# babybirdprd/dia-tts-prune

Measured on AMD Instinct MI355X. Metric: audio-codec frames/sec (Dia-1.6B decode, whole job), higher is better.
Workload: dtype bf16; 1 GPU; Dia-1.6B bf16 weights, bf16 K/V, batch 1, 1890 decode steps, text bytes [98], cfg 3.0 / T 1.3 / top-p 0.95 / top-k 35, hipGraph=True; batch_per_gpu=1, parallelism=single

## Files before the change

dia-tts-prune_amd/csrc/seg.hip:

```cpp
#include "common.hpp"
#include "../../include/dia_hip.h"
#include "errors.hpp"
#include "launch.hpp"
#include "tuning.hpp"

namespace {

constexpr int SG_CUS = 256;
constexpr int SG_NCW = 7;
constexpr int SG_NT = (SG_NCW + 1) * 64;
constexpr int SG_TILES = 16;
constexpr int SG_K = 2048;
constexpr int SG_D = 2048, SG_F = 8192, SG_NQ = 3072;
constexpr int SG_S_CO = SG_D / SG_CUS / 4;
constexpr int SG_S_WI = 2 * SG_F / SG_CUS / 4;
constexpr int SG_S_WO = 8;
constexpr int SG_S_QKV = SG_NQ / SG_CUS / 4;
constexpr int SG_FIRST_WI = SG_S_CO, SG_FIRST_WO = SG_S_CO + SG_S_WI, SG_FIRST_QKV = SG_FIRST_WO + SG_S_WO;
constexpr int SG_SLOTS_FULL = SG_FIRST_QKV + SG_S_QKV;
constexpr int SG_KMAX = (SG_SLOTS_FULL + SG_NCW - 1) / SG_NCW;
constexpr int SG_MAXM = 4;

constexpr int SG_CNT_STRIDE = 16;
constexpr int SG_CNT_X1 = 0, SG_CNT_H = 8, SG_CNT_P = 16, SG_CNT_X2 = 80, SG_NCNT = 88;
constexpr size_t SG_OFF_LAUNCH = (size_t)SG_NCNT * SG_CNT_STRIDE * 4;
constexpr size_t SG_OFF_ERR = SG_OFF_LAUNCH + SG_CUS * 4;
constexpr size_t SG_CTRL_BYTES = (SG_OFF_ERR + 64 + 255) / 256 * 256;
constexpr size_t SG_OFF_V1 = SG_CTRL_BYTES;
constexpr size_t SG_OFF_X1 = SG_OFF_V1 + SG_MAXM * SG_D * 4;
constexpr size_t SG_OFF_SSQ1 = SG_OFF_X1 + SG_MAXM * SG_D * 4;
constexpr size_t SG_OFF_H = SG_OFF_SSQ1 + SG_MAXM * SG_CUS * 4;
constexpr size_t SG_OFF_P = SG_OFF_H + 4 * SG_MAXM * SG_K * 4;
constexpr size_t SG_OFF_V2 = SG_OFF_P + 64 * 3 * SG_MAXM * 32 * 4;
constexpr size_t SG_OFF_SSQ2 = SG_OFF_V2 + SG_MAXM * SG_D * 4;
constexpr size_t SG_WS_BYTES = SG_OFF_SSQ2 + SG_MAXM * 64 * 4;

constexpr size_t SG_L_PLANES = 0;
constexpr size_t SG_L_RAW = SG_L_PLANES + 3 * SG_TILES * 64 * 16;
constexpr size_t SG_L_PART = SG_L_RAW + SG_MAXM * SG_K * 4;
constexpr size_t SG_L_MISC = SG_L_PART + 16 * 16 * 16;
constexpr size_t SG_LDS_BYTES = SG_L_MISC + 64;

struct SegK {
  const float* a_in; int a_ktiles;
  const bf16_raw* W; int nslots; int M; int has_qkv;
  float* x; int ldx;
  const float* g_mlp; const float* g_next;
  float* qkv_out; int ldq;
  float* planes_x; int xkt; float* ssq; int ssq_ld;
  float inv_d, eps;
  unsigned char* ws;
  long long timeout_ticks;
  int dbg;
  int head_sleep;
  long long* stamps;
};

__device__ __forceinline__ long long sg_clock() { return (long long)__builtin_amdgcn_s_memrealtime(); }

__device__ __forceinline__ void sg_bar() { lds_barrier(); }

__device__ __forceinline__ int sg_op_of(int s) { return s < SG_FIRST_WI ? 0 : (s < SG_FIRST_WO ? 1 : (s < SG_FIRST_QKV ? 2 : 3)); }
__device__ __forceinline__ int sg_op_first(int op) { return op == 0 ? 0 : (op == 1 ? SG_FIRST_WI : (op == 2 ? SG_FIRST_WO : SG_FIRST_QKV)); }

__device__ __forceinline__ void sg_convert(unsigned char* smem, int tid, int M) {
  const float* raw = reinterpret_cast<const float*>(smem + SG_L_RAW);
  bf16x8* planes = reinterpret_cast<bf16x8*>(smem + SG_L_PLANES);
#pragma unroll
  for (int u = 0; u < (SG_TILES * 64) / SG_NT; ++u) {
    const int i = tid + u * SG_NT;
    const int t = i >> 6, l = i & 63;
    const int r = l & 3, g = (l & 15) >> 2, q = l >> 4;
    if (r < M) {
      const float4* src = reinterpret_cast<const float4*>(raw + r * SG_K + 128 * t + 32 * g + 8 * q);
      bf16x8 h, mi, lo;
      split3x8(src[0], src[1], h, mi, lo);
      planes[i] = h; planes[SG_TILES * 64 + i] = mi; planes[2 * SG_TILES * 64 + i] = lo;
    }
  }
}

__device__ __forceinline__ void sg_load_slot(bf16x8 (&b)[SG_TILES], const bf16_raw* W, int cu, int nslots, int s, int lane, int dbg = 0) {
  if (dbg & 1) return;
  const bf16x8* src = reinterpret_cast<const bf16x8*>(W) + ((long)(cu * nslots + s) * SG_TILES) * 64 + lane;
#pragma unroll
  for (int t = 0; t < SG_TILES; ++t) b[t] = __builtin_nontemporal_load(src + t * 64);
}

__device__ __forceinline__ void sg_consume(const bf16x8 (&b)[SG_TILES], unsigned char* smem, int slot_in_op, int lane) {
  const bf16x8* planes = reinterpret_cast<const bf16x8*>(smem + SG_L_PLANES);
  f32x4 a0 = {0.f, 0.f, 0.f, 0.f}, a1 = a0, a2 = a0;
#pragma unroll
  for (int t = 0; t < SG_TILES; ++t) {
    const bf16x8 h = planes[t * 64 + lane], mi = planes[SG_TILES * 64 + t * 64 + lane], lo = planes[2 * SG_TILES * 64 + t * 64 + lane];
    a0 = __builtin_amdgcn_mfma_f32_16x16x32_bf16(h, b[t], a0, 0, 0, 0);
    a1 = __builtin_amdgcn_mfma_f32_16x16x32_bf16(mi, b[t], a1, 0, 0, 0);
    a2 = __builtin_amdgcn_mfma_f32_16x16x32_bf16(lo, b[t], a2, 0, 0, 0);
  }
  f32x4 a;
#pragma unroll
  for (int r = 0; r < 4; ++r) a[r] = (a0[r] + a1[r]) + a2[r];
  const int g = lane >> 4;
  if (((lane & 15) >> 2) == g) reinterpret_cast<f32x4*>(smem + SG_L_PART)[(slot_in_op * 4 + g) * 4 + (lane & 3)] = a;
}

__device__ __forceinline__ float sg_part(const unsigned char* smem, int slot_in_op, int c, int r) {
  const float* p = reinterpret_cast<const float*>(smem + SG_L_PART) + (slot_in_op * 16 + c) * 4 + r;
  return ((p[0] + p[16]) + p[32]) + p[48];
}

struct SgSync {
  unsigned char* ws; unsigned* err; int* abort_s; long long timeout; int lane;
  __device__ __forceinline__ unsigned* cnt(int i) const { return reinterpret_cast<unsigned*>(ws) + i * SG_CNT_STRIDE; }
  __device__ __forceinline__ void wait(int first, int n, unsigned want, unsigned code) const {
    if (*abort_s) return;
    const long long t0 = sg_clock();
    const unsigned* p = cnt(first + (lane < n ? lane : 0));
    for (;;) {
      const unsigned v = __hip_atomic_load(p, __ATOMIC_RELAXED, __HIP_MEMORY_SCOPE_AGENT);
      if (__all(lane >= n || v == want)) break;
      __builtin_amdgcn_s_sleep(2);
      if (sg_clock() - t0 > timeout) {
        if (lane == 0) { __hip_atomic_store(err, code, __ATOMIC_RELAXED, __HIP_MEMORY_SCOPE_AGENT); *abort_s = 1; }
        break;
      }
    }
    __builtin_amdgcn_fence(__ATOMIC_ACQUIRE, "wavefront");
  }
  __device__ __forceinline__ void arrive(int c) const {
    asm volatile("s_waitcnt vmcnt(0)" ::: "memory");
    if (lane == 0) __hip_atomic_fetch_add(cnt(c), 1u, __ATOMIC_RELAXED, __HIP_MEMORY_SCOPE_AGENT);
  }
};

__device__ __forceinline__ void st1_agent(float* p, float v) { __hip_atomic_store(p, v, __ATOMIC_RELAXED, __HIP_MEMORY_SCOPE_AGENT); }
__device__ __forceinline__ float ld1_agent(const float* p) { return __hip_atomic_load(p, __ATOMIC_RELAXED, __HIP_MEMORY_SCOPE_AGENT); }

__device__ __forceinline__ void sg_gather_rows(const float* src, int ld, int M, unsigned char* smem, int lane) {
  const __amdgpu_buffer_rsrc_t r = agent_rsrc(src);
  float4* raw = reinterpret_cast<float4*>(smem + SG_L_RAW);
  f32x4 v[SG_MAXM * 8];
#pragma unroll
  for (int u = 0; u < SG_MAXM * 8; ++u) {
    const int row = min(u >> 3, M - 1), c = (u & 7) * 64 + lane;
    v[u] = ld4_agent(r, (row * ld + c * 4) * 4);
  }
#pragma unroll
  for (int u = 0; u < SG_MAXM * 8; ++u) {
    const int row = u >> 3, c = (u & 7) * 64 + lane;
    if (row < M) raw[row * (SG_K / 4) + c] = float4{v[u][0], v[u][1], v[u][2], v[u][3]};
  }
}

template <int SG_NB>
__global__ __launch_bounds__(SG_NT) void k_seg_mlp(SegK p) {
  extern __shared__ __attribute__((aligned(16))) unsigned char smem[];
  const int tid = threadIdx.x, lane = tid & 63, w = tid >> 6, cu = blockIdx.x;
  const int M = p.M, nslots = p.nslots;
  const int nops = p.has_qkv ? 4 : 3;
  float* inv_s = reinterpret_cast<float*>(smem + SG_L_MISC);
  int* abort_s = reinterpret_cast<int*>(smem + SG_L_MISC + 32);

  if (w < SG_NCW) {
    bf16x8 buf[SG_NB][SG_TILES];
    for (int i = 0; i < (w >= SG_S_CO ? 2 * p.head_sleep : p.head_sleep); ++i) __builtin_amdgcn_s_sleep(1);
#pragma unroll
    for (int k = 0; k < SG_NB; ++k) {
      const int s = w + SG_NCW * k;
      if (s < nslots) sg_load_slot(buf[k], p.W, cu, nslots, s, lane, p.dbg);
    }
    {
      bf16x8* planes = reinterpret_cast<bf16x8*>(smem + SG_L_PLANES);
      const bf16x8 z = {0, 0, 0, 0, 0, 0, 0, 0};
      for (int i = tid; i < SG_TILES * 64; i += SG_NCW * 64)
        if ((i & 3) >= M) { planes[i] = z; planes[SG_TILES * 64 + i] = z; planes[2 * SG_TILES * 64 + i] = z; }
    }
    int cur = -1;
    auto advance_to = [&](int op) {
      while (cur < op) {
        if (cur >= 0) sg_bar();
        sg_bar();
        sg_convert(smem, tid, M);
        sg_bar();
        ++cur;
      }
    };
#pragma unroll
    for (int k = 0; k < SG_KMAX; ++k) {
      const int s = w + SG_NCW * k;
      if (s < nslots) {
        const int op = sg_op_of(s);
        advance_to(op);
        sg_consume(buf[k % SG_NB], smem, s - sg_op_first(op), lane);
        const int s2 = s + SG_NCW * SG_NB;
        if (s2 < nslots) sg_load_slot(buf[k % SG_NB], p.W, cu, nslots, s2, lane, p.dbg);
      }
    }
    advance_to(nops - 1);
    sg_bar();
    return;
  }

  SgSync sy{p.ws, reinterpret_cast<unsigned*>(p.ws + SG_OFF_ERR), abort_s, p.timeout_ticks, lane};
  if (lane == 0) *abort_s = 0;
  unsigned* launch_no = reinterpret_cast<unsigned*>(p.ws + SG_OFF_LAUNCH);
  const unsigned L1 = launch_no[cu] + 1u;
  float* v1 = reinterpret_cast<float*>(p.ws + SG_OFF_V1);
  float* x1b = reinterpret_cast<float*>(p.ws + SG_OFF_X1);
  float* ssq1 = reinterpret_cast<float*>(p.ws + SG_OFF_SSQ1);
  float* hb = reinterpret_cast<float*>(p.ws + SG_OFF_H);
  float* pb = reinterpret_cast<float*>(p.ws + SG_OFF_P);
  float* v2 = reinterpret_cast<float*>(p.ws + SG_OFF_V2);
  float* ssq2 = reinterpret_cast<float*>(p.ws + SG_OFF_SSQ2);

#define SG_STAMP(i) do { if (p.stamps && lane == 0) p.stamps[cu * 16 + (i)] = sg_clock(); } while (0)
  SG_STAMP(0);
  const int r8 = lane >> 3, c8 = lane & 7;
  const bool live8 = r8 < M;
  const int n8 = 8 * cu + c8;
  const float xold = p.x[(long)(live8 ? r8 : 0) * p.ldx + n8];
  const float gm = p.g_mlp[n8];
  {
    float4* raw = reinterpret_cast<float4*>(smem + SG_L_RAW);
    float4 fa[SG_MAXM * 4], fb[SG_MAXM * 4];
#pragma unroll
    for (int u = 0; u < SG_MAXM * 4; ++u) {
      const int f = u * 64 + lane, row = min(f >> 8, M - 1), idx = f & 255, kt = idx >> 2, q = idx & 3;
      const float4* src = reinterpret_cast<const float4*>(p.a_in + ((long)kt * 64 + row + 16 * q) * 8);
      fa[u] = src[0]; fb[u] = src[1];
    }
#pragma unroll
    for (int u = 0; u < SG_MAXM * 4; ++u) {
      const int f = u * 64 + lane, row = f >> 8, idx = f & 255;
      if (row < M) { raw[row * (SG_K / 4) + idx * 2] = fa[u]; raw[row * (SG_K / 4) + idx * 2 + 1] = fb[u]; }
    }
  }
  SG_STAMP(1);
  sg_bar();
  sg_convert(smem, tid, M);
  sg_bar();
  SG_STAMP(2);
  sg_bar();
  SG_STAMP(3);

  {
    float x1 = 0.f;
    if (live8) {
      x1 = xold + sg_part(smem, c8 >> 2, c8 & 3, r8);
      st1_agent(x1b + r8 * SG_D + n8, x1);
      st1_agent(v1 + r8 * SG_D + n8, mul_rn(x1, gm));
    }
    float sq = mul_rn(x1, x1);
    sq += __shfl_xor(sq, 1, 64); sq += __shfl_xor(sq, 2, 64); sq += __shfl_xor(sq, 4, 64);
    if (live8 && c8 == 0) st1_agent(ssq1 + r8 * SG_CUS + cu, sq);
    sy.arrive(SG_CNT_X1 + (cu & 7));
  }
  SG_STAMP(4);
  sy.wait(SG_CNT_X1, 8, 32u * L1, 1u);
  SG_STAMP(5);
  float x1own = 0.f;
  float x1own2 = 0.f;
  {
    sg_gather_rows(v1, SG_D, M, smem, lane);
    const __amdgpu_buffer_rsrc_t sr = agent_rsrc(ssq1);
#pragma unroll
    for (int r = 0; r < SG_MAXM; ++r) {
      if (r < M) {
        const f32x4 q = ld4_agent(sr, (r * SG_CUS + lane * 4) * 4);
        const float s = wave_sum((q[0] + q[1]) + (q[2] + q[3]));
        if (lane == 0) inv_s[r] = rsqrtf(s * p.inv_d + p.eps);
      }
    }
    if (cu < 64) {
      const int e0 = lane, e1 = lane + 64;
      if (e0 < M * 32) x1own = ld1_agent(x1b + (e0 >> 5) * SG_D + 32 * cu + (e0 & 31));
      if (e1 < M * 32) x1own2 = ld1_agent(x1b + (e1 >> 5) * SG_D + 32 * cu + (e1 & 31));
    }
  }
  SG_STAMP(6);
  sg_bar();
  sg_convert(smem, tid, M);
  sg_bar();
  sg_bar();
  SG_STAMP(7);

  {
    const int quarter = cu >> 6;
#pragma unroll
    for (int u = 0; u < 2; ++u) {
      const int e = lane + 64 * u, r = e >> 5, hcol = e & 31;
      if (e < M * 32) {
        const float inv = inv_s[r];
        const float g = sg_part(smem, hcol >> 2, hcol & 3, r) * inv, up = sg_part(smem, 8 + (hcol >> 2), hcol & 3, r) * inv;
        st1_agent(hb + ((long)quarter * SG_MAXM + r) * SG_K + 32 * (cu & 63) + hcol, (g / (1.0f + expf(-g))) * up);
      }
    }
    sy.arrive(SG_CNT_H + quarter);
    SG_STAMP(8);
    sy.wait(SG_CNT_H + quarter, 1, 64u * L1, 2u);
    SG_STAMP(9);
    sg_gather_rows(hb + (long)quarter * SG_MAXM * SG_K, SG_K, M, smem, lane);
  }
  sg_bar();
  sg_convert(smem, tid, M);
  sg_bar();
  sg_bar();
  SG_STAMP(10);

  {
    const int quarter = cu >> 6, c = cu & 63;
    float acc[2];
#pragma unroll
    for (int u = 0; u < 2; ++u) {
      const int e = lane + 64 * u, r = e >> 5, col = e & 31;
      acc[u] = (e < M * 32) ? sg_part(smem, col >> 2, col & 3, r) : 0.f;
    }
    if (quarter != 0) {
#pragma unroll
      for (int u = 0; u < 2; ++u) {
        const int e = lane + 64 * u;
        if (e < M * 32) st1_agent(pb + ((long)(c * 3 + quarter - 1) * SG_MAXM + (e >> 5)) * 32 + (e & 31), acc[u]);
      }
      sy.arrive(SG_CNT_P + c);
    } else {
      sy.wait(SG_CNT_P + c, 1, 3u * L1, 3u);
#pragma unroll
      for (int u = 0; u < 2; ++u) {
        const int e = lane + 64 * u, r = e >> 5, col = e & 31;
        const bool live = e < M * 32;
        float x2 = 0.f;
        if (live) {
          const float p1 = ld1_agent(pb + ((long)(c * 3 + 0) * SG_MAXM + r) * 32 + col);
          const float p2 = ld1_agent(pb + ((long)(c * 3 + 1) * SG_MAXM + r) * 32 + col);
          const float p3 = ld1_agent(pb + ((long)(c * 3 + 2) * SG_MAXM + r) * 32 + col);
          const int n = 32 * c + col;
          x2 = (u == 0 ? x1own : x1own2) + (((acc[u] + p1) + p2) + p3);
          p.x[(long)r * p.ldx + n] = x2;
          const float vg = mul_rn(x2, p.g_next[n]);
          p.planes_x[plane_frag_off(r, n & ~7, p.xkt) + (n & 7)] = vg;
          if (p.has_qkv) st1_agent(v2 + r * SG_D + n, vg);
        }
        const float s16 = row16_sum(mul_rn(x2, x2));
        const float s32 = s16 + __shfl_xor(s16, 16, 64);
        if (live && (col & 15) == 0) p.ssq[(long)(2 * c + (col >> 4)) * p.ssq_ld + r] = s16;
        if (live && col == 0 && p.has_qkv) st1_agent(ssq2 + r * 64 + c, s32);
      }
      sy.arrive(SG_CNT_X2 + (c & 7));
    }
  }
  SG_STAMP(11);
  if (p.has_qkv) {
    sy.wait(SG_CNT_X2, 8, 8u * L1, 4u);
    SG_STAMP(12);
    sg_gather_rows(v2, SG_D, M, smem, lane);
#pragma unroll
    for (int r = 0; r < SG_MAXM; ++r) {
      if (r < M) {
        const float s = wave_sum(ld1_agent(ssq2 + r * 64 + lane));
        if (lane == 0) inv_s[r] = rsqrtf(s * p.inv_d + p.eps);
      }
    }
    SG_STAMP(13);
    sg_bar();
    sg_convert(smem, tid, M);
    sg_bar();
    sg_bar();
    SG_STAMP(14);
    const int r = lane / 12, cc = lane % 12;
    if (r < M) p.qkv_out[(long)r * p.ldq + 12 * cu + cc] = sg_part(smem, cc >> 2, cc & 3, r) * inv_s[r];
  }
  if (lane == 0) launch_no[cu] = L1;
  SG_STAMP(15);
}

}

extern "C" int64_t dia_seg_workspace_bytes(void) { return (int64_t)SG_WS_BYTES; }
extern "C" int64_t dia_seg_workspace_control_bytes(void) { return (int64_t)SG_CTRL_BYTES; }
extern "C" int32_t dia_seg_slots(int with_qkv) { return with_qkv ? SG_SLOTS_FULL : SG_FIRST_QKV; }

extern "C" int dia_seg_supported(int D, int F, int attn_width, int nqkv) {
  if (D != SG_D || F != SG_F || attn_width != SG_K || nqkv != SG_NQ) return 0;
  int dev = 0;
  hipDeviceProp_t pr;
  if (hipGetDevice(&dev) != hipSuccess || hipGetDeviceProperties(&pr, dev) != hipSuccess) return 0;
  return pr.multiProcessorCount >= SG_CUS ? 1 : 0;
}

extern "C" int dia_seg_error(const void* ws, void* stream) {
  if (!ws) return dia_fail(DIA_E_ARG, "dia_seg_error: null workspace");
  unsigned code = 0;
  hipError_t e = hipMemcpyAsync(&code, (const unsigned char*)ws + SG_OFF_ERR, 4, hipMemcpyDeviceToHost, (hipStream_t)stream);
  if (e == hipSuccess) e = hipStreamSynchronize((hipStream_t)stream);
  if (e != hipSuccess) return dia_fail_hip(e, "dia_seg_error");
  return (int)code;
}

extern "C" int dia_seg_mlp(const dia_seg_args* a, void* stream) {
  if (!a || !a->a_in || !a->W || !a->x || !a->g_mlp || !a->g_next || !a->planes_x || !a->ssq || !a->ws)
    return dia_fail(DIA_E_ARG, "dia_seg_mlp: null argument");
  if (a->M < 1 || a->M > SG_MAXM) return dia_fail(DIA_E_ARG, "dia_seg_mlp: 1..4 rows");
  if (a->D != SG_D || a->F != SG_F || a->a_ktiles * 32 != SG_K) return dia_fail(DIA_E_ARG, "dia_seg_mlp: built for D 2048, F 8192, attention width 2048");
  if (a->has_qkv && (!a->qkv_out || a->ldq < SG_NQ)) return dia_fail(DIA_E_ARG, "dia_seg_mlp: q/k/v output missing");
  if (a->nslots != (a->has_qkv ? SG_SLOTS_FULL : SG_FIRST_QKV)) return dia_fail(DIA_E_ARG, "dia_seg_mlp: slot count does not match the ring layout");
  if (a->xkt * 32 < SG_D || a->ssq_ld < a->M || a->ldx < SG_D) return dia_fail(DIA_E_ARG, "dia_seg_mlp: output layout too narrow");
  SegK k;
  k.a_in = a->a_in; k.a_ktiles = a->a_ktiles; k.W = (const bf16_raw*)a->W; k.nslots = a->nslots; k.M = a->M; k.has_qkv = a->has_qkv ? 1 : 0;
  k.x = a->x; k.ldx = a->ldx; k.g_mlp = a->g_mlp; k.g_next = a->g_next; k.qkv_out = a->qkv_out; k.ldq = a->ldq;
  k.planes_x = a->planes_x; k.xkt = a->xkt; k.ssq = a->ssq; k.ssq_ld = a->ssq_ld; k.inv_d = 1.0f / SG_D; k.eps = a->eps;
  k.ws = (unsigned char*)a->ws;
  k.stamps = (long long*)a->stamps;
  k.timeout_ticks = a->timeout_us > 0 ? (long long)a->timeout_us * 100 : 2000000LL;
  k.dbg = dia_tune(DIA_TUNE_SEG_DBG) > 0 ? dia_tune(DIA_TUNE_SEG_DBG) : 0;
  k.head_sleep = dia_tune(DIA_TUNE_SEG_SLEEP) >= 0 ? dia_tune(DIA_TUNE_SEG_SLEEP) : 8;
  const int nb = dia_tune(DIA_TUNE_SEG_NB) > 0 ? dia_tune(DIA_TUNE_SEG_NB) : 3;
  if (nb == 1) dia_launch<k_seg_mlp<1>>(dim3(SG_CUS), dim3(SG_NT), SG_LDS_BYTES, (hipStream_t)stream, k);
  else if (nb == 2) dia_launch<k_seg_mlp<2>>(dim3(SG_CUS), dim3(SG_NT), SG_LDS_BYTES, (hipStream_t)stream, k);
  else dia_launch<k_seg_mlp<3>>(dim3(SG_CUS), dim3(SG_NT), SG_LDS_BYTES, (hipStream_t)stream, k);
  return dia_check_launch("k_seg_mlp");
}
```

dia-tts-prune_amd/dia_hip/engine.py:

```python

from __future__ import annotations

import ctypes as C
from dataclasses import dataclass
from functools import partial
from typing import Dict, List, Optional, Sequence

import numpy as np
import torch

from . import binding as hb
from . import compact as cpt
from . import layout as lay
from .config import DiaConfig
from .pruning import is_2of4
from .quant import is_mxfp8

HEAD_DIM = 128
_TILERS = {1: lay.tile_weight, 2: lay.tile_weight_bf16x2, 3: lay.tile_weight_planes}


def _ceil(v: int, m: int) -> int:
    return (v + m - 1) // m * m

# ... 818 lines not shown
            return t

        if self.B > 1:
            from concurrent.futures import ThreadPoolExecutor
            with ThreadPoolExecutor(max_workers=min(self.B, 8)) as pool:
                parts = list(pool.map(draw, range(self.B)))
        else:
            parts = [draw(0)]
        host = torch.stack(parts)
        with torch.cuda.stream(self.stream):
            self.noise[:, r0:rows].copy_(host, non_blocking=False)
        self._noise_rows = rows

    def decode(self, n_steps: int, use_graph: bool = True):
        if not self.prefilled:
            raise hb.DiaHipError("decode() before prefill()")
        self.ensure_noise(self._issued + int(n_steps))
        self._enqueue_steps(int(n_steps), use_graph)
        self._issued += int(n_steps)

    def _enqueue_steps(self, n_steps: int, use_graph: bool):
        hb.check(hb.lib().dia_engine_decode(self._engine, int(n_steps), int(bool(use_graph))), "dia_engine_decode")

    def profile_step(self) -> np.ndarray:
        n = hb.lib().dia_engine_launches_per_step(self._engine)
        buf = (C.c_float * n)()
        self.ensure_noise(self._issued + 1)
        hb.check(hb.lib().dia_engine_profile_step(self._engine, buf, n), "dia_engine_profile_step")
        self._issued += 1
        return np.array(buf[:], dtype=np.float64)

    def launches_per_step(self) -> int:
        return int(hb.lib().dia_engine_launches_per_step(self._engine))

    def seg_error(self) -> int:
        if not self.seg:
            return 0
        return int(hb.lib().dia_seg_error(hb.ptr(self.seg_ws), C.c_void_p(self.stream.cuda_stream)))

    def time_step(self) -> np.ndarray:
        n = hb.lib().dia_engine_launches_per_step(self._engine)
        buf, ivl = (C.c_float * n)(), (C.c_float * n)()
        self.ensure_noise(self._issued + 1)
        got = hb.lib().dia_engine_time_step(self._engine, buf, ivl, n)
        if got < 0:
            hb.check(got, "dia_engine_time_step")
        self._issued += 1
        self.last_kernel_names = [hb.lib().dia_timed_kernel_name(i).decode() for i in range(got)]
        self.last_intervals_ms = np.array(ivl[:got], dtype=np.float64)
        return np.array(buf[:got], dtype=np.float64)

    def sync(self):
        self.stream.synchronize()
        self._pinned.clear()

    def steps_total(self) -> int:
        return self.max_tokens - self.prefill_step

    def run(self, use_graph: bool = True, poll: int = 64):
        remaining = self.steps_total()
        first = True
        while remaining > 0:
            n = min(8 if first else poll, remaining)
            first = False
            self.decode(n, use_graph)
            remaining -= n
            self.ensure_noise(self._issued + min(poll, remaining))
            self.sync()
            if self.seg and self.seg_error():
                self.results()
            if bool((self.fsm[:, 3] != 0).all().item()):
                break

    def logits_host(self) -> np.ndarray:
        self.sync()
        lg = self.logits[: self.R, : self.C * self.V].reshape(self.B, 2, self.C, self.V)
        return lg.cpu().numpy()

    def _raise_if_invalid(self):
        if int(self.mlp_barrier[1].item()) != 0:
            raise hb.DiaHipError("fused MLP kernel: a workgroup gave up waiting at the grid barrier; results are invalid")
        code = self.seg_error()
        if code:
            self.seg_ws[: int(hb.lib().dia_seg_workspace_control_bytes())].zero_()
            raise hb.DiaHipError(f"persistent MLP segment: an in-kernel wait timed out (code {code}: 1 x1, 2 hidden, 3 wo partials, "
                                 f"4 x2) — were all 256 workgroups resident?  Results are invalid; set DIA_TUNE=seg=0 to run the launches")

    def results(self) -> List[UtteranceResult]:
        self.sync()
        self._raise_if_invalid()
        tok = self.tokens.cpu().numpy()
        prd = self.pred.cpu().numpy()
        fsm = self.fsm.cpu().numpy()
        cur = self.cur.cpu().numpy()
        out = []
        for b in range(self.B):
            last = int(fsm[b, 4]) if fsm[b, 3] else int(cur[b]) - 1
            out.append(UtteranceResult(tok[b], tok[b, self.first_steps[b]: last + 1].copy(), last, prd[b], self.lens[b]))
        return out

    @classmethod
    def open(cls, w: DeviceWeights, slots: int, *, s_cap: Optional[int] = None, kv_dtype: str = "bf16",
             max_tokens: Optional[int] = None, ignore_eos: bool = False, stream: Optional[torch.cuda.Stream] = None,
             cfg_scale: float = 3.0, temperature: float = 1.3, top_p: float = 0.95, top_k: int = 35,
             attention: str = "auto") -> "DecodeSession":
        if int(slots) < 1:
            raise ValueError("slots must be >= 1")
        if float(temperature) == 0.0:
            temperature = 1.0
        cap = w.cfg.data.text_length if s_cap is None else int(s_cap)
        if not (1 <= cap <= w.cfg.data.text_length):
            raise ValueError(f"s_cap must be in [1, {w.cfg.data.text_length}]")
        empty = np.zeros((0,), dtype=np.int32)
        s = cls(w, [empty] * int(slots), kv_dtype=kv_dtype, max_tokens=max_tokens, cfg_scale=cfg_scale, temperature=temperature,
                top_p=top_p, top_k=top_k, ignore_eos=ignore_eos, stream=stream, s_cap=_ceil(cap, 32), attention=attention,
                _slotted=True)
        s.text_cap = cap
        return s

    def _init_slots(self):
        B, dev, sp = self.B, self.dev, self.sample_params
        self.text_cap = self.S
        self.slot_f32 = [torch.full((B,), float(sp[k]), dtype=torch.float32).to(dev) for k in ("cfg_scale", "temperature", "top_p")]
        self.slot_i32 = [torch.full((B,), int(v), dtype=torch.int32).to(dev) for v in (sp["top_k"], self.max_tokens)]
        fsm = np.zeros((B, 8), dtype=np.int32)
        fsm[:, 1], fsm[:, 2], fsm[:, 3] = -1, self.max_delay, 1
        self.fsm = torch.from_numpy(fsm).to(dev)
        self._gens = None
        self._live: Dict[int, dict] = {}
        self._parked = set(range(B))

    def free_slots(self) -> List[int]:
        return [b for b in range(self.B) if b not in self._live]

    def _as_request(self, r) -> Request:
        if not isinstance(r, Request):
            r = Request(np.asarray(r, dtype=np.int32))
        mt = self.max_tokens if r.max_tokens is None else int(r.max_tokens)
        ids = np.asarray(r.text_ids, dtype=np.int32).reshape(-1)
        if len(ids) > self.text_cap:
            raise ValueError(f"request text of {len(ids)} bytes exceeds the session's s_cap = {self.text_cap}")
        if not (2 <= mt <= self.T):
            raise ValueError(f"max_tokens must be in [2, {self.T}]")
        if mt > self.max_tokens:
            raise ValueError(f"max_tokens {mt} exceeds the session's {self.max_tokens} (the noise buffer's steps per slot)")
        pr = r.audio_prompt
        if pr is not None:
            pr = np.asarray(pr)
            if pr.ndim == 3 and pr.shape[0] == 1:
                pr = pr[0]
            if pr.ndim != 2 or pr.shape[1] != self.C:
                raise ValueError(f"Unexpected audio_prompt shape: {pr.shape}. Expected [T, C] or [1, T, C].")
            if 1 + pr.shape[0] + self.max_delay > self.T:
                raise ValueError(f"audio prompt of {pr.shape[0]} frames does not fit audio_length {self.T}")
        return Request(ids, r.seed, mt, float(r.cfg_scale), float(r.temperature), float(r.top_p), int(r.top_k or 0), pr)

    def admit(self, requests: Sequence) -> List[int]:
        if not self.slotted:
            raise hb.DiaHipError("admit() needs a session made by DecodeSession.open()")
        reqs = [self._as_request(r) for r in requests]
        free = self.free_slots()
        if len(reqs) > len(free):
            raise hb.DiaHipError(f"admit(): {len(reqs)} requests for {len(free)} free slots")
        pairs = list(zip(free, reqs))
        for i in range(0, len(pairs), hb.SLOTS_PER_CALL):
            self._admit(pairs[i: i + hb.SLOTS_PER_CALL])
        return [b for b, _ in pairs]
# ... 170 lines not shown
```

scratch/seg_stamps.py:

```python
import ctypes as C, sys, os
ROOT = os.path.dirname(os.path.dirname(os.path.abspath(__file__)))
sys.path.insert(0, os.path.join(ROOT, "dia-tts-prune_amd")); sys.path.insert(0, os.path.join(ROOT, "tests"))
import numpy as np, torch
from dia_hip import binding as hb, layout as lay
import test_gpu_seg as T

M = int(sys.argv[1]) if len(sys.argv) > 1 else 2
dev = torch.device("cuda:0")
L = hb.lib()
W, a, x0, g_mlp, g_next = T.make_case(M, 1, True, dev)
rings = [lay.seg_ring(W["co"], W["gate"], W["up"], W["wo"], W["qkv"]) for _ in range(1)]
rings += [rings[0].clone() for _ in range(11)]
a_t = lay.pack_f32_tiles(a, ktiles=64, mtiles=1)
x = torch.zeros(16, 2048, device=dev); x[:M] = x0
planes_x = torch.zeros(3, 1, 64, 64, 8, dtype=torch.bfloat16, device=dev)
ssq = torch.zeros(128, 16, device=dev); qkv = torch.zeros(16, 3072, device=dev)
ws = torch.zeros(int(L.dia_seg_workspace_bytes()), dtype=torch.uint8, device=dev)
stamps = torch.zeros(256, 16, dtype=torch.int64, device=dev)
def args(ring, st):
    s = hb.SegArgs()
    s.a_in, s.a_ktiles, s.M, s.W, s.nslots, s.has_qkv, s.D, s.F = hb.ptr(a_t), 64, M, hb.ptr(ring), 29, 1, 2048, 8192
    s.x, s.ldx, s.g_mlp, s.g_next, s.qkv_out, s.ldq = hb.ptr(x), 2048, hb.ptr(g_mlp), hb.ptr(g_next), hb.ptr(qkv), 3072
    s.planes_x, s.xkt, s.ssq, s.ssq_ld, s.eps, s.ws = hb.ptr(planes_x), 64, hb.ptr(ssq), 16, 1e-5, hb.ptr(ws)
    s.stamps = hb.ptr(st) if st is not None else None
    return s
big = torch.randn(8192, 8192, device=dev)
for _ in range(40):
    big = (big @ big) * 1e-4
torch.cuda.synchronize()
for i in range(3000):
    hb.check(L.dia_seg_mlp(C.byref(args(rings[i % 12], None)), None), "seg")
torch.cuda.synchronize()
ev0, ev1 = torch.cuda.Event(enable_timing=True), torch.cuda.Event(enable_timing=True)
for rep in range(3):
    ev0.record()
    for i in range(24):
        hb.check(L.dia_seg_mlp(C.byref(args(rings[i % 12], stamps if i == 23 else None)), None), "seg")
    ev1.record(); torch.cuda.synchronize()
    print(f"24 eager launches: {ev0.elapsed_time(ev1) / 24 * 1e3:.2f} us per launch (host-paced)")
assert L.dia_seg_error(hb.ptr(ws), None) == 0
st = stamps.cpu().numpy().astype(np.float64) / 100.0
t0 = st[:, 0].min()
names = ["start", "attn rows in LDS", "planes(co) ready", "co computed", "x1 published", "x1 complete (all CUs)", "x1 gathered",
         "wi computed", "h published", "h quarter complete", "wo computed", "wo partial out / reduced+x2 published", "x2 complete", "x2 gathered",
         "qkv computed", "end"]
print(f"{'phase':42s} {'min':>7s} {'median':>7s} {'max':>7s}   (us after the first workgroup's start; reducers = CUs 0..63)")
for i, nme in enumerate(names):
    v = st[:, i] - t0
    print(f"{i:2d} {nme:39s} {v.min():7.2f} {np.median(v):7.2f} {v.max():7.2f}")
```

Measured before the change: 1032 frames/s.

## Replace counter barriers with launch-tagged 64-bit values in persistent MLP segment

```diff
diff --git a/dia-tts-prune_amd/csrc/seg.hip b/dia-tts-prune_amd/csrc/seg.hip
--- a/dia-tts-prune_amd/csrc/seg.hip
+++ b/dia-tts-prune_amd/csrc/seg.hip
@@ -21,19 +21,17 @@
 constexpr int SG_KMAX = (SG_SLOTS_FULL + SG_NCW - 1) / SG_NCW;
 constexpr int SG_MAXM = 4;
 
-constexpr int SG_CNT_STRIDE = 16;
-constexpr int SG_CNT_X1 = 0, SG_CNT_H = 8, SG_CNT_P = 16, SG_CNT_X2 = 80, SG_NCNT = 88;
-constexpr size_t SG_OFF_LAUNCH = (size_t)SG_NCNT * SG_CNT_STRIDE * 4;
+constexpr size_t SG_OFF_LAUNCH = 0;
 constexpr size_t SG_OFF_ERR = SG_OFF_LAUNCH + SG_CUS * 4;
 constexpr size_t SG_CTRL_BYTES = (SG_OFF_ERR + 64 + 255) / 256 * 256;
 constexpr size_t SG_OFF_V1 = SG_CTRL_BYTES;
-constexpr size_t SG_OFF_X1 = SG_OFF_V1 + SG_MAXM * SG_D * 4;
-constexpr size_t SG_OFF_SSQ1 = SG_OFF_X1 + SG_MAXM * SG_D * 4;
-constexpr size_t SG_OFF_H = SG_OFF_SSQ1 + SG_MAXM * SG_CUS * 4;
-constexpr size_t SG_OFF_P = SG_OFF_H + 4 * SG_MAXM * SG_K * 4;
-constexpr size_t SG_OFF_V2 = SG_OFF_P + 64 * 3 * SG_MAXM * 32 * 4;
-constexpr size_t SG_OFF_SSQ2 = SG_OFF_V2 + SG_MAXM * SG_D * 4;
-constexpr size_t SG_WS_BYTES = SG_OFF_SSQ2 + SG_MAXM * 64 * 4;
+constexpr size_t SG_OFF_X1 = SG_OFF_V1 + SG_MAXM * SG_D * 8;
+constexpr size_t SG_OFF_SSQ1 = SG_OFF_X1 + SG_MAXM * SG_D * 8;
+constexpr size_t SG_OFF_H = SG_OFF_SSQ1 + SG_MAXM * SG_CUS * 8;
+constexpr size_t SG_OFF_P = SG_OFF_H + 4 * SG_MAXM * SG_K * 8;
+constexpr size_t SG_OFF_V2 = SG_OFF_P + 64 * 3 * SG_MAXM * 32 * 8;
+constexpr size_t SG_OFF_SSQ2 = SG_OFF_V2 + SG_MAXM * SG_D * 8;
+constexpr size_t SG_WS_BYTES = SG_OFF_SSQ2 + SG_MAXM * 64 * 8;
 
 constexpr size_t SG_L_PLANES = 0;
 constexpr size_t SG_L_RAW = SG_L_PLANES + 3 * SG_TILES * 64 * 16;
@@ -42,19 +40,14 @@
 constexpr size_t SG_LDS_BYTES = SG_L_MISC + 64;
 
 struct SegK {
-  const float* a_in; int a_ktiles;
-  const bf16_raw* W; int nslots; int M; int has_qkv;
-  float* x; int ldx;
-  const float* g_mlp; const float* g_next;
+  const float* g_next;
   float* qkv_out; int ldq;
   float* planes_x; int xkt; float* ssq; int ssq_ld;
   float inv_d, eps;
-  unsigned char* ws;
   long long timeout_ticks;
-  int dbg;
-  int head_sleep;
   long long* stamps;
 };
+constexpr int SG_FLAG_QKV = 1, SG_FLAG_STAMPS = 2, SG_FLAG_DBG_SHIFT = 8, SG_FLAG_SLEEP_SHIFT = 16;
 
 __device__ __forceinline__ long long sg_clock() { return (long long)__builtin_amdgcn_s_memrealtime(); }
 
@@ -109,65 +102,78 @@
   return ((p[0] + p[16]) + p[32]) + p[48];
 }
 
+typedef unsigned long long sg_u64;
+typedef unsigned sg_u32x2 __attribute__((ext_vector_type(2)));
+
+__device__ __forceinline__ void sg_publish(unsigned char* ws, size_t off, int idx, unsigned tag, float v) {
+  __hip_atomic_store(reinterpret_cast<sg_u64*>(ws + off) + idx, ((sg_u64)tag << 32) | (sg_u64)__float_as_uint(v), __ATOMIC_RELAXED,
+                     __HIP_MEMORY_SCOPE_AGENT);
+}
+
 struct SgSync {
-  unsigned char* ws; unsigned* err; int* abort_s; long long timeout; int lane;
-  __device__ __forceinline__ unsigned* cnt(int i) const { return reinterpret_cast<unsigned*>(ws) + i * SG_CNT_STRIDE; }
-  __device__ __forceinline__ void wait(int first, int n, unsigned want, unsigned code) const {
-    if (*abort_s) return;
-    const long long t0 = sg_clock();
-    const unsigned* p = cnt(first + (lane < n ? lane : 0));
+  __amdgpu_buffer_rsrc_t ws; unsigned* err; long long timeout; unsigned tag; int lane; bool dead;
+  __device__ __forceinline__ sg_u32x2 ld(int byte_off) const { return __builtin_amdgcn_raw_buffer_load_b64(ws, byte_off, 0, 16); }
+  __device__ __forceinline__ bool expired(long long& t0, unsigned code) {
+    __builtin_amdgcn_s_sleep(1);
+    const long long t = sg_clock();
+    if (t0 == 0) t0 = t;
+    if (t - t0 <= timeout) return false;
+    if (lane == 0) __hip_atomic_store(err, code, __ATOMIC_RELAXED, __HIP_MEMORY_SCOPE_AGENT);
+    dead = true;
+    return true;
+  }
+  __device__ __forceinline__ void sweep_rows(int off, int rows, unsigned char* smem, unsigned code) {
+    float* raw = reinterpret_cast<float*>(smem + SG_L_RAW);
+    long long t0 = 0;
+    for (int r = 0; r < rows; ++r) {
+      const int o = off + (r * SG_K + lane) * 8;
+      sg_u32x2 v[SG_K / 64];
+      for (;;) {
+#pragma unroll
+        for (int k = 0; k < SG_K / 64; ++k) v[k] = ld(o + k * 512);
+        bool ok = true;
+#pragma unroll
+        for (int k = 0; k < SG_K / 64; ++k) ok &= v[k][1] == tag;
+        if (__all(ok) || dead || expired(t0, code)) break;
+      }
+#pragma unroll
+      for (int k = 0; k < SG_K / 64; ++k) raw[r * SG_K + k * 64 + lane] = __uint_as_float(v[k][0]);
+    }
+  }
+  template <int N>
+  __device__ __forceinline__ void sweep(const int (&off)[N], float (&out)[N], unsigned code) {
+    long long t0 = 0;
+    sg_u32x2 v[N];
     for (;;) {
-      const unsigned v = __hip_atomic_load(p, __ATOMIC_RELAXED, __HIP_MEMORY_SCOPE_AGENT);
-      if (__all(lane >= n || v == want)) break;
-      __builtin_amdgcn_s_sleep(2);
-      if (sg_clock() - t0 > timeout) {
-        if (lane == 0) { __hip_atomic_store(err, code, __ATOMIC_RELAXED, __HIP_MEMORY_SCOPE_AGENT); *abort_s = 1; }
-        break;
-      }
-    }
-    __builtin_amdgcn_fence(__ATOMIC_ACQUIRE, "wavefront");
-  }
-  __device__ __forceinline__ void arrive(int c) const {
-    asm volatile("s_waitcnt vmcnt(0)" ::: "memory");
-    if (lane == 0) __hip_atomic_fetch_add(cnt(c), 1u, __ATOMIC_RELAXED, __HIP_MEMORY_SCOPE_AGENT);
+#pragma unroll
+      for (int k = 0; k < N; ++k) v[k] = ld(off[k]);
+      bool ok = true;
+#pragma unroll
+      for (int k = 0; k < N; ++k) ok &= v[k][1] == tag;
+      if (__all(ok) || dead || expired(t0, code)) break;
+    }
+#pragma unroll
+    for (int k = 0; k < N; ++k) out[k] = __uint_as_float(v[k][0]);
   }
 };
 
-__device__ __forceinline__ void st1_agent(float* p, float v) { __hip_atomic_store(p, v, __ATOMIC_RELAXED, __HIP_MEMORY_SCOPE_AGENT); }
-__device__ __forceinline__ float ld1_agent(const float* p) { return __hip_atomic_load(p, __ATOMIC_RELAXED, __HIP_MEMORY_SCOPE_AGENT); }
-
-__device__ __forceinline__ void sg_gather_rows(const float* src, int ld, int M, unsigned char* smem, int lane) {
-  const __amdgpu_buffer_rsrc_t r = agent_rsrc(src);
-  float4* raw = reinterpret_cast<float4*>(smem + SG_L_RAW);
-  f32x4 v[SG_MAXM * 8];
-#pragma unroll
-  for (int u = 0; u < SG_MAXM * 8; ++u) {
-    const int row = min(u >> 3, M - 1), c = (u & 7) * 64 + lane;
-    v[u] = ld4_agent(r, (row * ld + c * 4) * 4);
-  }
-#pragma unroll
-  for (int u = 0; u < SG_MAXM * 8; ++u) {
-    const int row = u >> 3, c = (u & 7) * 64 + lane;
-    if (row < M) raw[row * (SG_K / 4) + c] = float4{v[u][0], v[u][1], v[u][2], v[u][3]};
-  }
-}
-
 template <int SG_NB>
-__global__ __launch_bounds__(SG_NT) void k_seg_mlp(SegK p) {
+__global__ __launch_bounds__(SG_NT) void k_seg_mlp(const float* a_in, float* x, const float* g_mlp, const bf16_raw* W, unsigned char* ws,
+                                                   int ldx, int nslots, int M, int a_flags, SegK p) {
   extern __shared__ __attribute__((aligned(16))) unsigned char smem[];
-  const int tid = threadIdx.x, lane = tid & 63, w = tid >> 6, cu = blockIdx.x;
-  const int M = p.M, nslots = p.nslots;
-  const int nops = p.has_qkv ? 4 : 3;
+  const int tid = threadIdx.x, lane = tid & 63, w = __builtin_amdgcn_readfirstlane(tid >> 6), cu = blockIdx.x;
+  const bool has_qkv = a_flags & SG_FLAG_QKV;
+  const int nops = has_qkv ? 4 : 3;
   float* inv_s = reinterpret_cast<float*>(smem + SG_L_MISC);
-  int* abort_s = reinterpret_cast<int*>(smem + SG_L_MISC + 32);
 
   if (w < SG_NCW) {
+    const int dbg = (a_flags >> SG_FLAG_DBG_SHIFT) & 0xff, head_sleep = (unsigned)a_flags >> SG_FLAG_SLEEP_SHIFT;
     bf16x8 buf[SG_NB][SG_TILES];
-    for (int i = 0; i < (w >= SG_S_CO ? 2 * p.head_sleep : p.head_sleep); ++i) __builtin_amdgcn_s_sleep(1);
+    for (int i = 0; i < (w >= SG_S_CO ? 2 * head_sleep : head_sleep); ++i) __builtin_amdgcn_s_sleep(1);
 #pragma unroll
     for (int k = 0; k < SG_NB; ++k) {
       const int s = w + SG_NCW * k;
-      if (s < nslots) sg_load_slot(buf[k], p.W, cu, nslots, s, lane, p.dbg);
+      if (s < nslots) sg_load_slot(buf[k], W, cu, nslots, s, lane, dbg);
     }
     {
       bf16x8* planes = reinterpret_cast<bf16x8*>(smem + SG_L_PLANES);
@@ -193,7 +199,7 @@
         advance_to(op);
         sg_consume(buf[k % SG_NB], smem, s - sg_op_first(op), lane);
         const int s2 = s + SG_NCW * SG_NB;
-        if (s2 < nslots) sg_load_slot(buf[k % SG_NB], p.W, cu, nslots, s2, lane, p.dbg);
+        if (s2 < nslots) sg_load_slot(buf[k % SG_NB], W, cu, nslots, s2, lane, dbg);
       }
     }
     advance_to(nops - 1);
@@ -201,40 +207,36 @@
     return;
   }
 
-  SgSync sy{p.ws, reinterpret_cast<unsigned*>(p.ws + SG_OFF_ERR), abort_s, p.timeout_ticks, lane};
-  if (lane == 0) *abort_s = 0;
-  unsigned* launch_no = reinterpret_cast<unsigned*>(p.ws + SG_OFF_LAUNCH);
-  const unsigned L1 = launch_no[cu] + 1u;
-  float* v1 = reinterpret_cast<float*>(p.ws + SG_OFF_V1);
-  float* x1b = reinterpret_cast<float*>(p.ws + SG_OFF_X1);
-  float* ssq1 = reinterpret_cast<float*>(p.ws + SG_OFF_SSQ1);
-  float* hb = reinterpret_cast<float*>(p.ws + SG_OFF_H);
-  float* pb = reinterpret_cast<float*>(p.ws + SG_OFF_P);
-  float* v2 = reinterpret_cast<float*>(p.ws + SG_OFF_V2);
-  float* ssq2 = reinterpret_cast<float*>(p.ws + SG_OFF_SSQ2);
-
-#define SG_STAMP(i) do { if (p.stamps && lane == 0) p.stamps[cu * 16 + (i)] = sg_clock(); } while (0)
-  SG_STAMP(0);
+  const bool stamping = a_flags & SG_FLAG_STAMPS;
+  const long long t_start = stamping ? sg_clock() : 0;
+#define SG_STAMP(i) do { if (stamping && lane == 0) p.stamps[cu * 16 + (i)] = sg_clock(); } while (0)
   const int r8 = lane >> 3, c8 = lane & 7;
   const bool live8 = r8 < M;
   const int n8 = 8 * cu + c8;
-  const float xold = p.x[(long)(live8 ? r8 : 0) * p.ldx + n8];
-  const float gm = p.g_mlp[n8];
+  const float xold = x[(long)(live8 ? r8 : 0) * ldx + n8];
+  const float gm = g_mlp[n8];
+  unsigned* launch_no = reinterpret_cast<unsigned*>(ws + SG_OFF_LAUNCH);
+  const unsigned ln = __hip_atomic_load(launch_no + cu, __ATOMIC_RELAXED, __HIP_MEMORY_SCOPE_AGENT);
   {
-    float4* raw = reinterpret_cast<float4*>(smem + SG_L_RAW);
-    float4 fa[SG_MAXM * 4], fb[SG_MAXM * 4];
+    f32x4* raw = reinterpret_cast<f32x4*>(smem + SG_L_RAW);
+    f32x4 fa[SG_MAXM * 4], fb[SG_MAXM * 4];
 #pragma unroll
     for (int u = 0; u < SG_MAXM * 4; ++u) {
       const int f = u * 64 + lane, row = min(f >> 8, M - 1), idx = f & 255, kt = idx >> 2, q = idx & 3;
-      const float4* src = reinterpret_cast<const float4*>(p.a_in + ((long)kt * 64 + row + 16 * q) * 8);
+      const f32x4* src = reinterpret_cast<const f32x4*>(a_in + ((long)kt * 64 + row + 16 * q) * 8);
       fa[u] = src[0]; fb[u] = src[1];
     }
+    __builtin_amdgcn_sched_barrier(0);
+    asm volatile("" :: "s"(p.g_next), "s"(p.qkv_out), "s"(p.ldq), "s"(p.planes_x), "s"(p.xkt), "s"(p.ssq), "s"(p.ssq_ld), "s"(p.inv_d),
+                 "s"(p.eps), "s"(p.timeout_ticks), "s"(p.stamps));
+    __builtin_amdgcn_sched_barrier(0);
 #pragma unroll
     for (int u = 0; u < SG_MAXM * 4; ++u) {
       const int f = u * 64 + lane, row = f >> 8, idx = f & 255;
-      if (row < M) { raw[row * (SG_K / 4) + idx * 2] = fa[u]; raw[row * (SG_K / 4) + idx * 2 + 1] = fb[u]; }
-    }
-  }
+      raw[row * (SG_K / 4) + idx * 2] = fa[u]; raw[row * (SG_K / 4) + idx * 2 + 1] = fb[u];
+    }
+  }
+  if (stamping && lane == 0) p.stamps[cu * 16] = t_start;
   SG_STAMP(1);
   sg_bar();
   sg_convert(smem, tid, M);
@@ -242,40 +244,48 @@
   SG_STAMP(2);
   sg_bar();
   SG_STAMP(3);
+
+  unsigned L1 = (unsigned)__builtin_amdgcn_readfirstlane((int)ln) + 1u;
+  if (L1 == 0u) L1 = 1u;
+  SgSync sy{agent_rsrc(ws), reinterpret_cast<unsigned*>(ws + SG_OFF_ERR), p.timeout_ticks, L1, lane, false};
 
   {
     float x1 = 0.f;
     if (live8) {
       x1 = xold + sg_part(smem, c8 >> 2, c8 & 3, r8);
-      st1_agent(x1b + r8 * SG_D + n8, x1);
-      st1_agent(v1 + r8 * SG_D + n8, mul_rn(x1, gm));
+      sg_publish(ws, SG_OFF_V1, r8 * SG_D + n8, L1, mul_rn(x1, gm));
+      sg_publish(ws, SG_OFF_X1, r8 * SG_D + n8, L1, x1);
     }
     float sq = mul_rn(x1, x1);
     sq += __shfl_xor(sq, 1, 64); sq += __shfl_xor(sq, 2, 64); sq += __shfl_xor(sq, 4, 64);
-    if (live8 && c8 == 0) st1_agent(ssq1 + r8 * SG_CUS + cu, sq);
-    sy.arrive(SG_CNT_X1 + (cu & 7));
+    if (live8 && c8 == 0) sg_publish(ws, SG_OFF_SSQ1, r8 * SG_CUS + cu, L1, sq);
   }
   SG_STAMP(4);
-  sy.wait(SG_CNT_X1, 8, 32u * L1, 1u);
-  SG_STAMP(5);
   float x1own = 0.f;
   float x1own2 = 0.f;
   {
-    sg_gather_rows(v1, SG_D, M, smem, lane);
-    const __amdgpu_buffer_rsrc_t sr = agent_rsrc(ssq1);
+    sy.sweep_rows((int)SG_OFF_V1, M, smem, 1u);
+    SG_STAMP(5);
+    int off[SG_MAXM * 4 + 2];
+    float val[SG_MAXM * 4 + 2];
+#pragma unroll
+    for (int r = 0; r < SG_MAXM; ++r)
+#pragma unroll
+      for (int j = 0; j < 4; ++j) off[r * 4 + j] = (int)SG_OFF_SSQ1 + (min(r, M - 1) * SG_CUS + lane * 4 + j) * 8;
+#pragma unroll
+    for (int u = 0; u < 2; ++u) {
+      const int e = lane + 64 * u, ec = e < M * 32 ? e : (e & 31);
+      off[SG_MAXM * 4 + u] = (int)SG_OFF_X1 + ((ec >> 5) * SG_D + 32 * (cu & 63) + (ec & 31)) * 8;
+    }
+    sy.sweep(off, val, 1u);
 #pragma unroll
     for (int r = 0; r < SG_MAXM; ++r) {
       if (r < M) {
-        const f32x4 q = ld4_agent(sr, (r * SG_CUS + lane * 4) * 4);
-        const float s = wave_sum((q[0] + q[1]) + (q[2] + q[3]));
+        const float s = wave_sum((val[r * 4] + val[r * 4 + 1]) + (val[r * 4 + 2] + val[r * 4 + 3]));
         if (lane == 0) inv_s[r] = rsqrtf(s * p.inv_d + p.eps);
       }
     }
-    if (cu < 64) {
-      const int e0 = lane, e1 = lane + 64;
-      if (e0 < M * 32) x1own = ld1_agent(x1b + (e0 >> 5) * SG_D + 32 * cu + (e0 & 31));
-      if (e1 < M * 32) x1own2 = ld1_agent(x1b + (e1 >> 5) * SG_D + 32 * cu + (e1 & 31));
-    }
+    x1own = val[SG_MAXM * 4]; x1own2 = val[SG_MAXM * 4 + 1];
   }
   SG_STAMP(6);
   sg_bar();
@@ -292,14 +302,12 @@
       if (e < M * 32) {
         const float inv = inv_s[r];
         const float g = sg_part(smem, hcol >> 2, hcol & 3, r) * inv, up = sg_part(smem, 8 + (hcol >> 2), hcol & 3, r) * inv;
-        st1_agent(hb + ((long)quarter * SG_MAXM + r) * SG_K + 32 * (cu & 63) + hcol, (g / (1.0f + expf(-g))) * up);
-      }
-    }
-    sy.arrive(SG_CNT_H + quarter);
+        sg_publish(ws, SG_OFF_H, (quarter * SG_MAXM + r) * SG_K + 32 * (cu & 63) + hcol, L1, (g / (1.0f + expf(-g))) * up);
+      }
+    }
     SG_STAMP(8);
-    sy.wait(SG_CNT_H + quarter, 1, 64u * L1, 2u);
+    sy.sweep_rows((int)SG_OFF_H + quarter * SG_MAXM * SG_K * 8, M, smem, 2u);
     SG_STAMP(9);
-    sg_gather_rows(hb + (long)quarter * SG_MAXM * SG_K, SG_K, M, smem, lane);
   }
   sg_bar();
   sg_convert(smem, tid, M);
@@ -319,44 +327,51 @@
 #pragma unroll
       for (int u = 0; u < 2; ++u) {
         const int e = lane + 64 * u;
-        if (e < M * 32) st1_agent(pb + ((long)(c * 3 + quarter - 1) * SG_MAXM + (e >> 5)) * 32 + (e & 31), acc[u]);
-      }
-      sy.arrive(SG_CNT_P + c);
+        if (e < M * 32) sg_publish(ws, SG_OFF_P, ((c * 3 + quarter - 1) * SG_MAXM + (e >> 5)) * 32 + (e & 31), L1, acc[u]);
+      }
     } else {
-      sy.wait(SG_CNT_P + c, 1, 3u * L1, 3u);
+      int off[6];
+      float part[6];
+#pragma unroll
+      for (int u = 0; u < 2; ++u) {
+        const int e = lane + 64 * u, ec = e < M * 32 ? e : (e & 31);
+#pragma unroll
+        for (int q = 0; q < 3; ++q) off[u * 3 + q] = (int)SG_OFF_P + (((c * 3 + q) * SG_MAXM + (ec >> 5)) * 32 + (ec & 31)) * 8;
+      }
+      sy.sweep(off, part, 3u);
 #pragma unroll
       for (int u = 0; u < 2; ++u) {
         const int e = lane + 64 * u, r = e >> 5, col = e & 31;
         const bool live = e < M * 32;
         float x2 = 0.f;
         if (live) {
-          const float p1 = ld1_agent(pb + ((long)(c * 3 + 0) * SG_MAXM + r) * 32 + col);
-          const float p2 = ld1_agent(pb + ((long)(c * 3 + 1) * SG_MAXM + r) * 32 + col);
-          const float p3 = ld1_agent(pb + ((long)(c * 3 + 2) * SG_MAXM + r) * 32 + col);
           const int n = 32 * c + col;
-          x2 = (u == 0 ? x1own : x1own2) + (((acc[u] + p1) + p2) + p3);
-          p.x[(long)r * p.ldx + n] = x2;
+          x2 = (u == 0 ? x1own : x1own2) + (((acc[u] + part[u * 3]) + part[u * 3 + 1]) + part[u * 3 + 2]);
+          x[(long)r * ldx + n] = x2;
           const float vg = mul_rn(x2, p.g_next[n]);
           p.planes_x[plane_frag_off(r, n & ~7, p.xkt) + (n & 7)] = vg;
-          if (p.has_qkv) st1_agent(v2 + r * SG_D + n, vg);
+          if (has_qkv) sg_publish(ws, SG_OFF_V2, r * SG_D + n, L1, vg);
         }
         const float s16 = row16_sum(mul_rn(x2, x2));
         const float s32 = s16 + __shfl_xor(s16, 16, 64);
         if (live && (col & 15) == 0) p.ssq[(long)(2 * c + (col >> 4)) * p.ssq_ld + r] = s16;
-        if (live && col == 0 && p.has_qkv) st1_agent(ssq2 + r * 64 + c, s32);
-      }
-      sy.arrive(SG_CNT_X2 + (c & 7));
+        if (live && col == 0 && has_qkv) sg_publish(ws, SG_OFF_SSQ2, r * 64 + c, L1, s32);
+      }
     }
   }
   SG_STAMP(11);
-  if (p.has_qkv) {
-    sy.wait(SG_CNT_X2, 8, 8u * L1, 4u);
+  if (has_qkv) {
+    sy.sweep_rows((int)SG_OFF_V2, M, smem, 4u);
     SG_STAMP(12);
-    sg_gather_rows(v2, SG_D, M, smem, lane);
+    int off[SG_MAXM];
+    float val[SG_MAXM];
+#pragma unroll
+    for (int r = 0; r < SG_MAXM; ++r) off[r] = (int)SG_OFF_SSQ2 + (min(r, M - 1) * 64 + lane) * 8;
+    sy.sweep(off, val, 4u);
 #pragma unroll
     for (int r = 0; r < SG_MAXM; ++r) {
       if (r < M) {
-        const float s = wave_sum(ld1_agent(ssq2 + r * 64 + lane));
+        const float s = wave_sum(val[r]);
         if (lane == 0) inv_s[r] = rsqrtf(s * p.inv_d + p.eps);
       }
     }
@@ -405,17 +420,20 @@
   if (a->nslots != (a->has_qkv ? SG_SLOTS_FULL : SG_FIRST_QKV)) return dia_fail(DIA_E_ARG, "dia_seg_mlp: slot count does not match the ring layout");
   if (a->xkt * 32 < SG_D || a->ssq_ld < a->M || a->ldx < SG_D) return dia_fail(DIA_E_ARG, "dia_seg_mlp: output layout too narrow");
   SegK k;
-  k.a_in = a->a_in; k.a_ktiles = a->a_ktiles; k.W = (const bf16_raw*)a->W; k.nslots = a->nslots; k.M = a->M; k.has_qkv = a->has_qkv ? 1 : 0;
-  k.x = a->x; k.ldx = a->ldx; k.g_mlp = a->g_mlp; k.g_next = a->g_next; k.qkv_out = a->qkv_out; k.ldq = a->ldq;
+  k.g_next = a->g_next; k.qkv_out = a->qkv_out; k.ldq = a->ldq;
   k.planes_x = a->planes_x; k.xkt = a->xkt; k.ssq = a->ssq; k.ssq_ld = a->ssq_ld; k.inv_d = 1.0f / SG_D; k.eps = a->eps;
-  k.ws = (unsigned char*)a->ws;
   k.stamps = (long long*)a->stamps;
   k.timeout_ticks = a->timeout_us > 0 ? (long long)a->timeout_us * 100 : 2000000LL;
-  k.dbg = dia_tune(DIA_TUNE_SEG_DBG) > 0 ? dia_tune(DIA_TUNE_SEG_DBG) : 0;
-  k.head_sleep = dia_tune(DIA_TUNE_SEG_SLEEP) >= 0 ? dia_tune(DIA_TUNE_SEG_SLEEP) : 8;
+  const int dbg = dia_tune(DIA_TUNE_SEG_DBG) > 0 ? dia_tune(DIA_TUNE_SEG_DBG) & 0xff : 0;
+  const int head_sleep = dia_tune(DIA_TUNE_SEG_SLEEP) >= 0 ? min(dia_tune(DIA_TUNE_SEG_SLEEP), 0x7fff) : 8;
+  const int flags = (a->has_qkv ? SG_FLAG_QKV : 0) | (a->stamps ? SG_FLAG_STAMPS : 0) | (dbg << SG_FLAG_DBG_SHIFT) | (head_sleep << SG_FLAG_SLEEP_SHIFT);
   const int nb = dia_tune(DIA_TUNE_SEG_NB) > 0 ? dia_tune(DIA_TUNE_SEG_NB) : 3;
-  if (nb == 1) dia_launch<k_seg_mlp<1>>(dim3(SG_CUS), dim3(SG_NT), SG_LDS_BYTES, (hipStream_t)stream, k);
-  else if (nb == 2) dia_launch<k_seg_mlp<2>>(dim3(SG_CUS), dim3(SG_NT), SG_LDS_BYTES, (hipStream_t)stream, k);
-  else dia_launch<k_seg_mlp<3>>(dim3(SG_CUS), dim3(SG_NT), SG_LDS_BYTES, (hipStream_t)stream, k);
+  const dim3 grid(SG_CUS), block(SG_NT);
+  const hipStream_t st = (hipStream_t)stream;
+  const bf16_raw* W = (const bf16_raw*)a->W;
+  unsigned char* ws = (unsigned char*)a->ws;
+  if (nb == 1) dia_launch<k_seg_mlp<1>>(grid, block, SG_LDS_BYTES, st, a->a_in, a->x, a->g_mlp, W, ws, a->ldx, a->nslots, a->M, flags, k);
+  else if (nb == 2) dia_launch<k_seg_mlp<2>>(grid, block, SG_LDS_BYTES, st, a->a_in, a->x, a->g_mlp, W, ws, a->ldx, a->nslots, a->M, flags, k);
+  else dia_launch<k_seg_mlp<3>>(grid, block, SG_LDS_BYTES, st, a->a_in, a->x, a->g_mlp, W, ws, a->ldx, a->nslots, a->M, flags, k);
   return dia_check_launch("k_seg_mlp");
 }
diff --git a/dia-tts-prune_amd/dia_hip/engine.py b/dia-tts-prune_amd/dia_hip/engine.py
--- a/dia-tts-prune_amd/dia_hip/engine.py
+++ b/dia-tts-prune_amd/dia_hip/engine.py
@@ -924,7 +924,7 @@
             raise hb.DiaHipError("fused MLP kernel: a workgroup gave up waiting at the grid barrier; results are invalid")
         code = self.seg_error()
         if code:
-            self.seg_ws[: int(hb.lib().dia_seg_workspace_control_bytes())].zero_()
+            self.seg_ws.zero_()
             raise hb.DiaHipError(f"persistent MLP segment: an in-kernel wait timed out (code {code}: 1 x1, 2 hidden, 3 wo partials, "
                                  f"4 x2) — were all 256 workgroups resident?  Results are invalid; set DIA_TUNE=seg=0 to run the launches")
 
diff --git a/scratch/seg_stamps.py b/scratch/seg_stamps.py
--- a/scratch/seg_stamps.py
+++ b/scratch/seg_stamps.py
@@ -41,8 +41,8 @@
 assert L.dia_seg_error(hb.ptr(ws), None) == 0
 st = stamps.cpu().numpy().astype(np.float64) / 100.0
 t0 = st[:, 0].min()
-names = ["start", "attn rows in LDS", "planes(co) ready", "co computed", "x1 published", "x1 complete (all CUs)", "x1 gathered",
-         "wi computed", "h published", "h quarter complete", "wo computed", "wo partial out / reduced+x2 published", "x2 complete", "x2 gathered",
+names = ["start", "attn rows in LDS", "planes(co) ready", "co computed", "x1 published", "x1 rows swept", "x1 ssq + own x1 swept",
+         "wi computed", "h published", "h quarter swept", "wo computed", "wo partial out / reduced+x2 published", "x2 rows swept", "x2 ssq swept",
          "qkv computed", "end"]
 print(f"{'phase':42s} {'min':>7s} {'median':>7s} {'max':>7s}   (us after the first workgroup's start; reducers = CUs 0..63)")
 for i, nme in enumerate(names):
```

New measurement: 1031 frames/s. About the same (-0.1%).
